# LIU-YUXI/SA-GNN

Measured on AMD Instinct MI355X. Metric: spmm_edges_per_sec, higher is better.
Workload: dtype f32

## Files before the change

sa-gnn_amd/csrc/attn_split.hip:

```cpp
#include "common.h"
#include "f16_split.h"

namespace {

typedef float f32x4 __attribute__((ext_vector_type(4)));
typedef int i32x4 __attribute__((ext_vector_type(4)));
typedef int i32x2 __attribute__((ext_vector_type(2)));

constexpr int kRows = 64;
constexpr int kBT = 4;
constexpr int kRec = 48;

template <int D>
__device__ __forceinline__ int swz(int row) {
  if (D == 128) return row & 15;
  if (D == 64) return (row >> 1) & 7;
  const int g = (row >> 2) & 3;
  return (0x78 >> (2 * g)) & 3;
}
__device__ __forceinline__ void lds_barrier() { asm volatile("s_waitcnt lgkmcnt(0)\n\ts_barrier" ::: "memory"); }

__host__ __device__ constexpr int pad_node(int t) { return t == 6 ? 16 : 0; }
__host__ __device__ constexpr int pad_group(int t) { return (t == 1 || t == 3 || t == 5) ? 64 : t == 6 ? 32 : 16; }
__host__ __device__ constexpr int lanes_per_pair(int t, int d) {
  if (d == 128) return (t % 4 == 0) ? 4 : (t % 2 == 0) ? 2 : 1;
  return t == 16 ? 4 : (t == 8 || t == 12) ? 2 : 1;
}

template <int DK>
struct HeadVec {
  typedef float type __attribute__((ext_vector_type(DK)));
  static __device__ __forceinline__ type load(const char* p, int gs) { return *reinterpret_cast<const type*>(p); }
  static __device__ __forceinline__ void store(char* p, int gs, type v) { *reinterpret_cast<type*>(p) = v; }
};
template <>
struct HeadVec<8> {
  typedef float type __attribute__((ext_vector_type(8)));
  typedef float f4 __attribute__((ext_vector_type(4)));
  static __device__ __forceinline__ type load(const char* p, int gs) {
    const f4 a = *reinterpret_cast<const f4*>(p), b = *reinterpret_cast<const f4*>(p + gs);
    return type{a[0], a[1], a[2], a[3], b[0], b[1], b[2], b[3]};
  }
  static __device__ __forceinline__ void store(char* p, int gs, type v) {
    *reinterpret_cast<f4*>(p) = f4{v[0], v[1], v[2], v[3]};
    *reinterpret_cast<f4*>(p + gs) = f4{v[4], v[5], v[6], v[7]};
  }
};

template <int CTRL>
__device__ __forceinline__ float dpp_add(float v) {
  return v + __builtin_bit_cast(float, __builtin_amdgcn_update_dpp(0, __builtin_bit_cast(int, v), CTRL, 0xf, 0xf, true));
}
template <int LPR>
__device__ __forceinline__ float row_sum(float v) {
  v = dpp_add<0xB1>(v);
  v = dpp_add<0x4E>(v);
  v = dpp_add<0x141>(v);
  if constexpr (LPR >= 16) v = dpp_add<0x140>(v);
  if constexpr (LPR == 32) v += __shfl_xor(v, 16);
  return v;
}

template <int D, int T, int LP, bool BWD>
__global__ __launch_bounds__(64 * (D >= 64 ? 4 : D / 16), (D == 128 || (BWD && T >= 8)) ? 1 : 2) void ln_mhsa_split_kernel(
    const float* __restrict__ x, int64_t ld_n, int64_t ld_t, int64_t n, const float* __restrict__ gamma,
    const float* __restrict__ beta, float eps, int apply_ln, const float* __restrict__ Wq,
    const float* __restrict__ bq, const float* __restrict__ Wk, const float* __restrict__ bk,
    const float* __restrict__ Wv, const float* __restrict__ bv, float* out, int64_t ld_out,
    int64_t n_tiles, float* __restrict__ dqkv_out, float* __restrict__ y_out, unsigned int* __restrict__ redo_ctr) {
  static_assert(!BWD || D <= 64 || LP == 1, "d = 128: the backward front keeps a pair in one lane");
  constexpr int NW = D >= 64 ? 4 : D / 16, NT = 64 * NW, KS = D / 32;
  constexpr int DK = D / 16;
  constexpr int HPW = 16 / DK;
  constexpr int NB = kRows / T;
  constexpr int ROWS = NB * T;
  constexpr int PLANE = kRows * D * 2;
  constexpr int LPR = D / 4, RPP = NT / LPR, NFILL = kRows / RPP;
  constexpr int PN = pad_node(T), PG = pad_group(T);
  constexpr int GS = kRows * kRec + NB * PN + PG;
  constexpr int QKVW = 4 * GS;
  typedef typename HeadVec<DK>::type vec;

  extern __shared__ __attribute__((aligned(16))) char lds[];
  char* const Yp = lds;
  char* const QKV = lds + 2 * PLANE;
  float2* const rstat = reinterpret_cast<float2*>(QKV + NW * QKVW);
  float2* const nstat = rstat + kRows;
  int* const flags = reinterpret_cast<int*>(nstat + NB);
  const int tid = threadIdx.x, lane = tid & 63;
  const int wave = __builtin_amdgcn_readfirstlane(tid >> 6);
  const int m = lane & 15, q = lane >> 4;
  const int cbase = 64 * (int)blockIdx.y + 16 * wave;
  const int col0 = cbase + 4 * q;
  const int fr = tid / LPR, fc4 = (tid % LPR) * 4;
  char* const tab = QKV + wave * QKVW;
  constexpr bool WL = D == 64 && (T & (T - 1)) == 0;
  constexpr int PP = T >= 4 ? T / 4 : 1;
  constexpr int GP = T >= 4 ? 4 : T;
  auto fill_row = [&](int p, int fr_now) { return WL ? 16 * wave + 4 * p + (lane >> 4) : p * RPP + fr_now; };

  float k4096 = 4096.f;
  asm volatile("" : "+v"(k4096));
  if (tid < 3) flags[tid] = 0;
  __syncthreads();
  const float qscale = 1.44269504088896340736f * (DK == 4 ? 0.5f : DK == 2 ? 0.70710678118654752440f : 0.35355339059327376220f);

  i32x4 wf[3][KS][2];
  {
    const float* const Ws[3] = {Wq, Wk, Wv};
    RangeTrack wr = range_init();
#pragma unroll
    for (int mat = 0; mat < 3; ++mat)
#pragma unroll
      for (int ks = 0; ks < KS; ++ks) {
        float wv[8];
#pragma unroll
        for (int j = 0; j < 8; ++j) wv[j] = Ws[mat][(size_t)(32 * ks + 8 * q + j) * D + cbase + m] * (mat == 0 ? qscale : 1.f);
        range_seg4(wr, wv[0], wv[1], wv[2], wv[3]);
        range_seg4(wr, wv[4], wv[5], wv[6], wv[7]);
#pragma unroll
        for (int e = 0; e < 4; ++e) {
          const int hd = head2(wv[2 * e], wv[2 * e + 1]);
          wf[mat][ks][0][e] = hd;
          wf[mat][ks][1][e] = tail2(hd, wv[2 * e], wv[2 * e + 1], k4096);
        }
      }
    if (range_bad(wr)) flags[2] = 1;
  }
  f32x4 bias3[3];
#pragma unroll
  for (int r = 0; r < 4; ++r) {
    bias3[0][r] = bq[col0 + r] * qscale;
    bias3[1][r] = bk[col0 + r];
    bias3[2][r] = bv[col0 + r];
  }
  float4 g4 = make_float4(1.f, 1.f, 1.f, 1.f), b4 = make_float4(0.f, 0.f, 0.f, 0.f);
  if (apply_ln) {
    g4 = *reinterpret_cast<const float4*>(gamma + fc4);
    b4 = *reinterpret_cast<const float4*>(beta + fc4);
  }
  const float inv_t = 1.f / (float)T;

  float4 xr[NFILL];
  auto fetch_tile = [&](int64_t tile) {
    const int64_t node0 = tile * NB;
#pragma unroll
    for (int p = 0; p < NFILL; ++p) {
      const int r = fill_row(p, fr);
      const int nb = r / T, ts = r - nb * T;
      xr[p] = make_float4(0.f, 0.f, 0.f, 0.f);
      if (tile < n_tiles && r < ROWS && node0 + nb < n)
        xr[p] = *reinterpret_cast<const float4*>(x + (node0 + nb) * ld_n + (int64_t)ts * ld_t + fc4);
    }
  };
  fetch_tile(blockIdx.x);

  int par = 0;
  for (int64_t tile = blockIdx.x; tile < n_tiles; tile += gridDim.x, par ^= 1) {
    const int64_t node0 = tile * NB;
    if (tid == 0) flags[par] = 0;
    int fr_ = fr, fc4_ = fc4, m_ = m, q_ = q;
    asm volatile("" : "+v"(fr_), "+v"(fc4_), "+v"(m_), "+v"(q_));

    float2 wst[NFILL];
    if constexpr (WL) {
      if (apply_ln) {
        float mr[NFILL], m2[NFILL];
#pragma unroll
        for (int p = 0; p < NFILL; ++p) {
          mr[p] = row_sum<LPR>((xr[p].x + xr[p].y) + (xr[p].z + xr[p].w)) * (1.f / (float)D);
          const float dx = xr[p].x - mr[p], dy = xr[p].y - mr[p], dz = xr[p].z - mr[p], dw = xr[p].w - mr[p];
          m2[p] = row_sum<LPR>((dx * dx + dy * dy) + (dz * dz + dw * dw));
        }
#pragma unroll
        for (int j = 0; j < NFILL / PP; ++j) {
          float sm = 0.f;
#pragma unroll
          for (int i = 0; i < PP; ++i) sm += mr[j * PP + i];
          if constexpr (GP >= 2) sm += __shfl_xor(sm, 16);
          if constexpr (GP == 4) sm += __shfl_xor(sm, 32);
          const float mean = sm * inv_t;
          float q2 = 0.f;
#pragma unroll
          for (int i = 0; i < PP; ++i) {
            const float dm = mr[j * PP + i] - mean;
            q2 += m2[j * PP + i] + (float)D * dm * dm;
          }
          if constexpr (GP >= 2) q2 += __shfl_xor(q2, 16);
          if constexpr (GP == 4) q2 += __shfl_xor(q2, 32);
          const float2 st = make_float2(mean, rsqrtf(q2 * (1.f / (float)(T * D)) + eps));
#pragma unroll
          for (int i = 0; i < PP; ++i) wst[j * PP + i] = st;
          const int r0 = fill_row(j * PP, fr_);
          if (fc4_ == 0 && r0 % T == 0) nstat[r0 / T] = st;
        }
      }
    } else if (apply_ln) {
#pragma unroll
      for (int p = 0; p < NFILL; ++p) {
        const float mr = row_sum<LPR>((xr[p].x + xr[p].y) + (xr[p].z + xr[p].w)) * (1.f / (float)D);
        const float dx = xr[p].x - mr, dy = xr[p].y - mr, dz = xr[p].z - mr, dw = xr[p].w - mr;
        const float m2 = row_sum<LPR>((dx * dx + dy * dy) + (dz * dz + dw * dw));
        if (fc4_ == 0) rstat[p * RPP + fr_] = make_float2(mr, m2);
      }
      lds_barrier();
      if (tid < NB) {
        float ms = 0.f;
#pragma unroll
        for (int ts = 0; ts < T; ++ts) ms += rstat[tid * T + ts].x;
        const float mean = ms * inv_t;
        float m2 = 0.f;
#pragma unroll
        for (int ts = 0; ts < T; ++ts) {
          const float2 st = rstat[tid * T + ts];
          const float dm = st.x - mean;
          m2 += st.y + (float)D * dm * dm;
        }
        nstat[tid] = make_float2(mean, rsqrtf(m2 * (1.f / (float)(T * D)) + eps));
      }
      lds_barrier();
    }
    RangeTrack yr = range_init();
#pragma unroll
    for (int p = 0; p < NFILL; ++p) {
      const int r = fill_row(p, fr_);
      float4 y = xr[p];
      if (apply_ln) {
        const float2 st = WL ? wst[p] : nstat[r < ROWS ? r / T : 0];
        const float ix = st.y * g4.x, iy = st.y * g4.y, iz = st.y * g4.z, iw = st.y * g4.w;
        y.x = xr[p].x * ix + (b4.x - st.x * ix);
        y.y = xr[p].y * iy + (b4.y - st.x * iy);
        y.z = xr[p].z * iz + (b4.z - st.x * iz);
        y.w = xr[p].w * iw + (b4.w - st.x * iw);
      }
      range_seg4(yr, y.x, y.y, y.z, y.w);
      if constexpr (BWD) {
        if (y_out && blockIdx.y == 0 && r < ROWS && node0 + r / T < n)
          *reinterpret_cast<float4*>(y_out + (node0 * T + r) * D + fc4_) = y;
      }
      const int p0 = head2(y.x, y.y), p1 = head2(y.z, y.w);
      const int off = r * (D * 2) + (((fc4_ >> 3) ^ swz<D>(r)) << 4) + ((fc4_ >> 2) & 1) * 8;
      *reinterpret_cast<i32x2*>(Yp + off) = i32x2{p0, p1};
      *reinterpret_cast<i32x2*>(Yp + PLANE + off) = i32x2{tail2(p0, y.x, y.y, k4096), tail2(p1, y.z, y.w, k4096)};
    }
    fetch_tile(tile + gridDim.x);
    lds_barrier();
    if (range_bad(yr)) flags[par] = 1;

#pragma unroll
    for (int bt = 0; bt < kBT; ++bt) {
      const int row = bt * 16 + m_;
      const int sw = swz<D>(row);
      f32x4 hi[3] = {bias3[0], bias3[1], bias3[2]};
      f32x4 lo[3];
#pragma unroll
      for (int ks = 0; ks < KS; ++ks) {
        const int off = row * (D * 2) + (((ks * 4 + q_) ^ sw) << 4);
        const f16x8 b1 = __builtin_bit_cast(f16x8, *reinterpret_cast<const i32x4*>(Yp + off));
        const f16x8 b2 = __builtin_bit_cast(f16x8, *reinterpret_cast<const i32x4*>(Yp + PLANE + off));
#pragma unroll
        for (int mat = 0; mat < 3; ++mat) {
          const f16x8 a1 = __builtin_bit_cast(f16x8, wf[mat][ks][0]);
          const f16x8 a2 = __builtin_bit_cast(f16x8, wf[mat][ks][1]);
          lo[mat] = __builtin_amdgcn_mfma_f32_16x16x32_f16(a2, b1, ks == 0 ? f32x4{0.f, 0.f, 0.f, 0.f} : lo[mat], 0, 0, 0);
          lo[mat] = __builtin_amdgcn_mfma_f32_16x16x32_f16(a1, b2, lo[mat], 0, 0, 0);
          hi[mat] = __builtin_amdgcn_mfma_f32_16x16x32_f16(a1, b1, hi[mat], 0, 0, 0);
        }
      }
      f32x4 acc[3];
#pragma unroll
      for (int mat = 0; mat < 3; ++mat)
#pragma unroll
        for (int r = 0; r < 4; ++r) acc[mat][r] = fmaf(lo[mat][r], kLoInv, hi[mat][r]);
      char* rec = tab + q_ * GS + row * kRec + (row / T) * PN;
      *reinterpret_cast<f32x4*>(rec) = acc[0];
      *reinterpret_cast<f32x4*>(rec + 16) = acc[1];
      *reinterpret_cast<f32x4*>(rec + 32) = acc[2];
    }
    lds_barrier();
    if (flags[par] | flags[2]) {
      if (tid == 0 && redo_ctr) atomicAdd(redo_ctr, 1u);
      constexpr int NCOL = 16 * NW;
      const float* const Ws[3] = {Wq, Wk, Wv};
      const float* const bs[3] = {bq, bk, bv};
      for (int idx = tid; idx < ROWS * 3 * NCOL; idx += NT) {
        const int r = idx / (3 * NCOL), rem = idx - r * (3 * NCOL), mat = rem / NCOL, cl = rem - mat * NCOL;
        const int nb = r / T, ts = r - nb * T;
        if (node0 + nb >= n) continue;
        const int col = 64 * (int)blockIdx.y + cl;
        const float sc = mat == 0 ? qscale : 1.f;
        const float2 st = apply_ln ? nstat[nb] : make_float2(0.f, 1.f);
        const float* const xrow = x + (node0 + nb) * ld_n + (int64_t)ts * ld_t;
        float acc = bs[mat][col] * sc;
        for (int k = 0; k < D; ++k) {
          float yv = xrow[k];
          if (apply_ln) {
            const float ik = st.y * gamma[k];
            yv = yv * ik + (beta[k] - st.x * ik);
          }
          acc = fmaf(yv, Ws[mat][(size_t)k * D + col] * sc, acc);
        }
        *reinterpret_cast<float*>(QKV + (cl >> 4) * QKVW + ((cl >> 2) & 3) * GS + r * kRec + nb * PN + mat * 16 + (cl & 3) * 4) = acc;
      }
      __syncthreads();
    }

    constexpr int PAIRS = NB * HPW;
    constexpr int LSTEP = 64 / LP;
    constexpr int TQ = T / LP;
    constexpr int KC = T <= 8 ? T : T / 2;
    static_assert(T % LP == 0 && T % KC == 0 && LP <= T, "query / key split");
    const int part = lane % LP;
    if constexpr (BWD) {
      const float scale = qscale * 0.69314718055994530942f;
      auto quad_sum = [&](float v) {
        if constexpr (LP > 1) v += __builtin_bit_cast(float, __builtin_amdgcn_update_dpp(0, __builtin_bit_cast(int, v), 0xB1, 0xf, 0xf, true));
        if constexpr (LP > 2) v += __builtin_bit_cast(float, __builtin_amdgcn_update_dpp(0, __builtin_bit_cast(int, v), 0x4E, 0xf, 0xf, true));
        return v;
      };
#pragma unroll 1
      for (int p = lane / LP; p < PAIRS; p += LSTEP) {
        const int hl = p % HPW, nb = p / HPW;
        const char* base = tab + ((hl * DK) >> 2) * GS + nb * (T * kRec + PN) + ((hl * DK) & 3) * 4;
        const int64_t node = node0 + nb;
        vec g = (vec)(0.f);
        if (node < n) g = *reinterpret_cast<const vec*>(out + node * ld_out + cbase + hl * DK);
        g *= inv_t;
        vec kv[T], vv[T], dk[T];
        float ps[T], asum[T];
#pragma unroll
        for (int ts = 0; ts < T; ++ts) {
          kv[ts] = HeadVec<DK>::load(base + ts * kRec + 16, GS);
          vv[ts] = HeadVec<DK>::load(base + ts * kRec + 32, GS);
          dk[ts] = (vec)(0.f);
          asum[ts] = 0.f;
          float pd = g[0] * vv[ts][0];
#pragma unroll
          for (int c = 1; c < DK; ++c) pd = fmaf(g[c], vv[ts][c], pd);
          ps[ts] = pd;
        }
        float* const drow = dqkv_out + (node * T) * (3 * D) + cbase + hl * DK;
#pragma unroll
        for (int i = 0; i < TQ; ++i) {
          const int tq = part * TQ + i;
          const vec qv = HeadVec<DK>::load(base + tq * kRec, GS);
          float a[T];
          float rs = 0.f;
#pragma unroll
          for (int s_ = 0; s_ < T; ++s_) {
            float z = qv[0] * kv[s_][0];
#pragma unroll
            for (int c = 1; c < DK; ++c) z = fmaf(qv[c], kv[s_][c], z);
            a[s_] = __builtin_amdgcn_exp2f(z);
            rs += a[s_];
          }
          const float inv = __builtin_amdgcn_rcpf(rs + 1e-8f);
          float dot = 0.f;
#pragma unroll
          for (int s_ = 0; s_ < T; ++s_) {
            a[s_] *= inv;
            dot = fmaf(a[s_], ps[s_], dot);
          }
          vec dq = (vec)(0.f);
#pragma unroll
          for (int s_ = 0; s_ < T; ++s_) {
            const float dz = a[s_] * (ps[s_] - dot);
            dq += dz * kv[s_];
            dk[s_] += dz * qv;
            asum[s_] += a[s_];
          }
          if (node < n) *reinterpret_cast<vec*>(drow + tq * (3 * D)) = dq * scale;
        }
        if constexpr (LP > 1) {
#pragma unroll
          for (int ts = 0; ts < T; ++ts) {
#pragma unroll
            for (int c = 0; c < DK; ++c) {
              float v = dk[ts][c];
              v = quad_sum(v);
              dk[ts][c] = v;
            }
            asum[ts] = quad_sum(asum[ts]);
          }
        }
        if (node < n) {
#pragma unroll
          for (int ts = 0; ts < T; ++ts) {
            if (LP > 1 && ts / TQ != part) continue;
            *reinterpret_cast<vec*>(drow + ts * (3 * D) + D) = dk[ts] * 0.69314718055994530942f;
            *reinterpret_cast<vec*>(drow + ts * (3 * D) + 2 * D) = g * asum[ts];
          }
        }
      }
      continue;
    }
#pragma unroll 1
    for (int p = lane / LP; p < PAIRS; p += LSTEP) {
      const int hl = p % HPW, nb = p / HPW;
      char* base = tab + ((hl * DK) >> 2) * GS + nb * (T * kRec + PN) + ((hl * DK) & 3) * 4;
      vec qv[TQ];
      float e[TQ][T], rs[TQ];
#pragma unroll
      for (int i = 0; i < TQ; ++i) qv[i] = HeadVec<DK>::load(base + (part * TQ + i) * kRec, GS);
#pragma unroll
      for (int ch = 0; ch < T / KC; ++ch) {
        vec k[KC];
#pragma unroll
        for (int s = 0; s < KC; ++s) k[s] = HeadVec<DK>::load(base + (ch * KC + s) * kRec + 16, GS);
#pragma unroll
        for (int i = 0; i < TQ; ++i)
#pragma unroll
          for (int s = 0; s < KC; ++s) {
            float pd = qv[i][0] * k[s][0];
#pragma unroll
            for (int c = 1; c < DK; ++c) pd = fmaf(qv[i][c], k[s][c], pd);
            const float ev = __builtin_amdgcn_exp2f(pd);
            e[i][ch * KC + s] = ev;
            rs[i] = (ch == 0 && s == 0) ? ev : rs[i] + ev;
          }
      }
      float w[T];
#pragma unroll
      for (int i = 0; i < TQ; ++i) {
        const float inv = __builtin_amdgcn_rcpf(rs[i] + 1e-8f);
#pragma unroll
        for (int s = 0; s < T; ++s) w[s] = i == 0 ? e[0][s] * inv : fmaf(e[i][s], inv, w[s]);
      }
      vec o = (vec)(0.f);
#pragma unroll
      for (int ch = 0; ch < T / KC; ++ch) {
        vec v[KC];
#pragma unroll
        for (int s = 0; s < KC; ++s) v[s] = HeadVec<DK>::load(base + (ch * KC + s) * kRec + 32, GS);
#pragma unroll
        for (int s = 0; s < KC; ++s) o += w[ch * KC + s] * v[s];
      }
      if (LP > 1) {
#pragma unroll
        for (int c = 0; c < DK; ++c) {
          float oc = o[c];
          oc += __builtin_bit_cast(float, __builtin_amdgcn_update_dpp(0, __builtin_bit_cast(int, oc), 0xB1, 0xf, 0xf, true));
          if (LP > 2) oc += __builtin_bit_cast(float, __builtin_amdgcn_update_dpp(0, __builtin_bit_cast(int, oc), 0x4E, 0xf, 0xf, true));
          o[c] = oc;
        }
      }
      const int64_t node = node0 + nb;
      if (part == 0 && node < n) {
        const vec ov = o * inv_t;
        float* dst = out + node * ld_out + cbase + hl * DK;
        if constexpr (DK == 8) {
          *reinterpret_cast<float4*>(dst) = make_float4(ov[0], ov[1], ov[2], ov[3]);
          *reinterpret_cast<float4*>(dst + 4) = make_float4(ov[4], ov[5], ov[6], ov[7]);
        } else {
          *reinterpret_cast<vec*>(dst) = ov;
        }
      }
    }
  }
}

}

namespace sagnn {

template <int D, int T, bool BWD>
static int launch_split(const SeqView& v, const AttnParams& a, float* out, int64_t ld_out, const AttnBwdOut& b, hipStream_t s) {
  constexpr int NW = D >= 64 ? 4 : D / 16, NB = kRows / T;
  constexpr int LP = (BWD && D == 128) ? 1 : lanes_per_pair(T, D);
  constexpr int GS = kRows * kRec + NB * pad_node(T) + pad_group(T);
  const size_t lds = (size_t)2 * kRows * D * 2 + (size_t)NW * 4 * GS + (size_t)(kRows + NB) * sizeof(float2) + 16;
  if (int rc = ensure_dynamic_lds(reinterpret_cast<const void*>(&ln_mhsa_split_kernel<D, T, LP, BWD>), lds)) return rc;
  const int per_cu = (D == 128 || (BWD && T >= 8)) ? 1 : D == 64 ? 2 : 4;
  constexpr int CB = D == 128 ? 2 : 1;
  const int64_t n_tiles = (v.n + NB - 1) / NB;
  const int64_t want = (int64_t)cu_count_current() * per_cu / CB;
  const int64_t blocks = n_tiles < want ? n_tiles : (want > 0 ? want : 1);
  ProfileScope prof(kProfMhsa, s, v.n, T);
  hipLaunchKernelGGL((ln_mhsa_split_kernel<D, T, LP, BWD>), dim3((unsigned)blocks, CB), dim3(64 * NW), lds, s, v.x, v.ld_n, v.ld_t,
                     v.n, a.gamma, a.beta, a.eps, a.apply_ln, a.Wq, a.bq, a.Wk, a.bk, a.Wv, a.bv,
                     BWD ? const_cast<float*>(b.g_out) : out, BWD ? b.ld_g : ld_out, n_tiles, b.dqkv, b.y, redo_counter());
  SAGNN_HIP_TRY(hipGetLastError());
  return SAGNN_OK;
}

template <int D>
static int ln_mhsa_mean_split_d(const SeqView& v, const AttnParams& a, float* out, int64_t ld_out, hipStream_t s) {
  int rc;
  const auto launch = [&](auto T) { return launch_split<D, decltype(T)::value, false>(v, a, out, ld_out, AttnBwdOut{}, s); };
  if (dispatch_t(v.t, SpecialisedT{}, launch, rc)) return rc;
  return fail(SAGNN_ERR_DIM, "split attention: t = %d has no specialised kernel", v.t);
}

int ln_mhsa_mean_split(const SeqView& v, const AttnParams& a, float* out, int64_t ld_out, hipStream_t s) {
  if (!mhsa_split_supported(v.d, v.t, a.heads)) return fail(SAGNN_ERR_DIM, "split attention: unsupported d/t/heads");
  if (v.d == 128) return ln_mhsa_mean_split_d<128>(v, a, out, ld_out, s);
  if (v.d == 64) return ln_mhsa_mean_split_d<64>(v, a, out, ld_out, s);
  return ln_mhsa_mean_split_d<32>(v, a, out, ld_out, s);
}

template <int D>
static int attn_bwd_front_split_d(const SeqView& v, const AttnParams& a, const AttnBwdOut& b, hipStream_t s) {
  using Ts = std::conditional_t<D == 128, SplitBwdFrontT128, SpecialisedT>;
  int rc;
  const auto launch = [&](auto T) { return launch_split<D, decltype(T)::value, true>(v, a, nullptr, 0, b, s); };
  if (dispatch_t(v.t, Ts{}, launch, rc)) return rc;
  return fail(SAGNN_ERR_DIM, "split attention backward front: t = %d has no specialised kernel", v.t);
}

int attn_bwd_front_split(const SeqView& v, const AttnParams& a, const AttnBwdOut& b, hipStream_t s) {
  if (!attn_bwd_front_split_supported(v.d, v.t, a.heads))
    return fail(SAGNN_ERR_DIM, "split attention backward front: unsupported d/t/heads");
  if (v.d == 128) return attn_bwd_front_split_d<128>(v, a, b, s);
  if (v.d == 64) return attn_bwd_front_split_d<64>(v, a, b, s);
  return attn_bwd_front_split_d<32>(v, a, b, s);
}

}
```

sa-gnn_amd/csrc/common.h:

```cpp
#pragma once
#include <hip/hip_runtime.h>
#include <stdint.h>
#include <stdio.h>
#include <string>

#include "engine.h"
#include "sagnn.h"

namespace sagnn {

std::string& last_error_slot();
int fail(int code, const char* fmt, ...) __attribute__((format(printf, 2, 3)));
int hip_fail(hipError_t e, const char* what);

inline bool aligned16(const void* p) { return (reinterpret_cast<uintptr_t>(p) & 15u) == 0; }

#define SAGNN_HIP_TRY(expr)                                   \
  do {                                                        \
    hipError_t _e = (expr);                                   \
    if (_e != hipSuccess) return ::sagnn::hip_fail(_e, #expr); \
  } while (0)

inline int lanes_per_row(int d) {
  int need = (d + 3) / 4;
  int lpr = 8;
  while (lpr < need) lpr <<= 1;
  return lpr;
}

int ensure_dynamic_lds(const void* kernel, size_t bytes);
int cu_count_current();
unsigned int* redo_counter();

struct SeqView {
  const float* x;
  int64_t ld_n, ld_t, n;
  int t, d;
  bool vec() const { return aligned16(x) && (ld_n & 3) == 0 && (ld_t & 3) == 0; }
};
struct AttnParams {
  int heads;
  const float *gamma, *beta;
  float eps;
  int apply_ln;
  const float *Wq, *bq, *Wk, *bk, *Wv, *bv;
};
struct AttnBwdOut {
  const float* g_out;
  int64_t ld_g;
  float *dqkv, *y;
};
struct LstmArgs {
  SeqView x;
  const float *W, *b;
  float forget_bias;
  const float* drop;
  float* h;
  int64_t ld_h;
  float *gates, *cell;
  const float* h_init;
  int64_t ld_hi;
  const float* c_init;
  float* c_final;
};

int lstm_fwd_mfma(const LstmArgs& a, hipStream_t s);
int ln_mhsa_mean_mfma(const SeqView& v, const AttnParams& a, float* out, int64_t ld_out, hipStream_t s);
int attn_bwd_front_mfma(const SeqView& v, const AttnParams& a, const AttnBwdOut& b, hipStream_t s);
int lstm_fwd_f16(const LstmArgs& a, hipStream_t s);
int ln_mhsa_mean_split(const SeqView& v, const AttnParams& a, float* out, int64_t ld_out, hipStream_t s);
int attn_bwd_front_split(const SeqView& v, const AttnParams& a, const AttnBwdOut& b, hipStream_t s);
int lstm_fwd_split128(const LstmArgs& a, hipStream_t s);
int attn_bwd_tail_f16(float* y, const float* dqkv, int64_t rows, int d, const float* Wqkv, float* dWqkv, float* dbqkv,
                      hipStream_t s);
int lstm_dw_f16(const float* x, int64_t ld_n, int64_t ld_t, const float* h, const float* dg, int64_t n, int t, int d, float* dW,
                hipStream_t s);
int dense_nn_any(const float* X, int64_t ldx, int64_t n, int din, int dout, const float* W, int64_t ldw,
                 const float* bias, float* Y, int64_t ldy, int accumulate, hipStream_t s);
int dense_tn_any(const float* X, int64_t ldx, const float* G, int64_t ldg, int64_t n, int din, int dout, float* dW,
                 int64_t lddw, float* db, hipStream_t s);
int gemm_nn(const float* X, int64_t ldx, int64_t n, int din, int dout, const float* W, int64_t ldw, const float* bias, float* Y,
            int64_t ldy, int accumulate, hipStream_t s);
int gemm_tn(const float* X, int64_t ldx, int64_t xseg, const float* G, int64_t ldg, int64_t gseg, int64_t seg_rows, int64_t n_seg,
            int din, int dout, float* dW, int64_t lddw, float* db, hipStream_t s);

enum ProfileKind { kProfSpmmRows = 0, kProfSpmmFixup = 1, kProfLstm = 2, kProfLayerNorm = 3, kProfMhsa = 4 };

class ProfileScope {
 public:
  ProfileScope(int kind, hipStream_t stream, int64_t units_a, int64_t units_b);
  ~ProfileScope();
  ProfileScope(const ProfileScope&) = delete;
  ProfileScope& operator=(const ProfileScope&) = delete;

 private:
  int slot_;
  hipStream_t stream_;
};

}
```

Measured before the change: 18.18 billion.

## Add specialised rows16 attention kernel for d=64, t=16 forward path

Adds a dedicated LayerNorm+MHSA mean kernel for d=64, t=16, 16 heads. Each wave holds one node's 16 timesteps and computes QKV with f16-split MFMA. Scores are formed with DPP row rotations in inline asm instead of going through LDS, and the kernel double-buffers tiles to run three workgroups per CU. Shared helpers move into a common header, and the split dispatcher routes this shape to the new kernel. This is aimed at the attention stage, which may not be what the spmm metric measures, and it adds hand-written asm with a fallback that recomputes when values fall out of range.

```diff
diff --git a/sa-gnn_amd/csrc/attn_rows16.hip b/sa-gnn_amd/csrc/attn_rows16.hip
--- /dev/null
+++ b/sa-gnn_amd/csrc/attn_rows16.hip
@@ -0,0 +1,276 @@
+#include "attn_split_common.h"
+
+#ifndef SAGNN_ROWS16_PER_CU
+#define SAGNN_ROWS16_PER_CU 3
+#endif
+
+namespace {
+
+constexpr int kD = 64, kT = 16;
+constexpr int kPlane = kRows * kD * 2;
+constexpr int kScratch = 3 * kT * kD * 4;
+constexpr int kLds = 4 * kPlane + kScratch + kBT * (int)sizeof(float2) + 16;
+constexpr int kLdsAsk = SAGNN_ROWS16_PER_CU >= 3 ? kLds : 160 * 1024 / (SAGNN_ROWS16_PER_CU + 1) + 1024;
+static_assert(kLdsAsk >= kLds && 3 * kLds <= 160 * 1024, "three workgroups per CU");
+
+template <int R>
+__device__ __forceinline__ float row_ror(float v) {
+  return __builtin_bit_cast(float, __builtin_amdgcn_update_dpp(0, __builtin_bit_cast(int, v), 0x120 + R, 0xf, 0xf, true));
+}
+
+#define SAGNN_DPP_ROW "row_mask:0xf bank_mask:0xf bound_ctrl:1\n\t"
+#define SAGNN_ROT_DOT(o, r)                                                  \
+  "v_mul_f32_dpp %" #o ", %15, %19 row_ror:" #r " " SAGNN_DPP_ROW            \
+  "v_fmac_f32_dpp %" #o ", %16, %20 row_ror:" #r " " SAGNN_DPP_ROW           \
+  "v_fmac_f32_dpp %" #o ", %17, %21 row_ror:" #r " " SAGNN_DPP_ROW           \
+  "v_fmac_f32_dpp %" #o ", %18, %22 row_ror:" #r " " SAGNN_DPP_ROW
+__device__ __forceinline__ void rotated_scores(const float (&q)[4], const float (&k)[4], float (&z)[kT]) {
+  z[0] = fmaf(k[3], q[3], fmaf(k[2], q[2], fmaf(k[1], q[1], k[0] * q[0])));
+  asm("s_nop 1\n\t"
+      SAGNN_ROT_DOT(0, 1) SAGNN_ROT_DOT(1, 2) SAGNN_ROT_DOT(2, 3) SAGNN_ROT_DOT(3, 4) SAGNN_ROT_DOT(4, 5)
+      SAGNN_ROT_DOT(5, 6) SAGNN_ROT_DOT(6, 7) SAGNN_ROT_DOT(7, 8) SAGNN_ROT_DOT(8, 9) SAGNN_ROT_DOT(9, 10)
+      SAGNN_ROT_DOT(10, 11) SAGNN_ROT_DOT(11, 12) SAGNN_ROT_DOT(12, 13) SAGNN_ROT_DOT(13, 14) SAGNN_ROT_DOT(14, 15)
+      : "=&v"(z[1]), "=&v"(z[2]), "=&v"(z[3]), "=&v"(z[4]), "=&v"(z[5]), "=&v"(z[6]), "=&v"(z[7]), "=&v"(z[8]), "=&v"(z[9]),
+        "=&v"(z[10]), "=&v"(z[11]), "=&v"(z[12]), "=&v"(z[13]), "=&v"(z[14]), "=&v"(z[15])
+      : "v"(k[0]), "v"(k[1]), "v"(k[2]), "v"(k[3]), "v"(q[0]), "v"(q[1]), "v"(q[2]), "v"(q[3]));
+}
+#undef SAGNN_ROT_DOT
+#undef SAGNN_DPP_ROW
+
+template <int... R>
+__device__ __forceinline__ float gather_weights(const float (&p)[kT], std::integer_sequence<int, R...>) {
+  float w = p[0];
+  ((w = row_ror<kT - 1 - R>(p[1 + R]) + w), ...);
+  return w;
+}
+__device__ __forceinline__ float key_weights(const float (&q)[4], const float (&k)[4]) {
+  float e[kT];
+  rotated_scores(q, k, e);
+  float rs = 0.f;
+#pragma unroll
+  for (int r = 0; r < kT; ++r) {
+    e[r] = __builtin_amdgcn_exp2f(e[r]);
+    rs = r == 0 ? e[0] : rs + e[r];
+  }
+  const float inv = __builtin_amdgcn_rcpf(rs + 1e-8f);
+#pragma unroll
+  for (int r = 0; r < kT; ++r) e[r] *= inv;
+  return gather_weights(e, std::make_integer_sequence<int, kT - 1>{});
+}
+
+__global__ __launch_bounds__(256, SAGNN_ROWS16_PER_CU) void ln_mhsa_rows16_kernel(
+    const float* __restrict__ x, int64_t ld_n, int64_t ld_t, int64_t n, const float* __restrict__ gamma,
+    const float* __restrict__ beta, float eps, int apply_ln, const float* __restrict__ Wq,
+    const float* __restrict__ bq, const float* __restrict__ Wk, const float* __restrict__ bk,
+    const float* __restrict__ Wv, const float* __restrict__ bv, float* out, int64_t ld_out,
+    int64_t n_tiles, unsigned int* __restrict__ redo_ctr) {
+  constexpr int D = kD, T = kT, KS = D / 32, NFILL = 4;
+
+  extern __shared__ __attribute__((aligned(16))) char lds[];
+  char* const Yp = lds;
+  float* const scratch = reinterpret_cast<float*>(lds + 4 * kPlane);
+  float2* const nstat = reinterpret_cast<float2*>(lds + 4 * kPlane + kScratch);
+  int* const flags = reinterpret_cast<int*>(nstat + kBT);
+  const int tid = threadIdx.x, lane = tid & 63;
+  const int wave = __builtin_amdgcn_readfirstlane(tid >> 6);
+  const int m = lane & 15, q = lane >> 4;
+  const int cbase = 16 * wave;
+  const int col0 = cbase + 4 * q;
+  const int fc4 = m * 4;
+
+  float k4096 = 4096.f;
+  asm volatile("" : "+v"(k4096));
+  if (tid < 4) flags[tid] = 0;
+  __syncthreads();
+  const float qscale = 1.44269504088896340736f * 0.5f;
+
+  i32x4 wf[3][KS][2];
+  {
+    const float* const Ws[3] = {Wq, Wk, Wv};
+    RangeTrack wr = range_init();
+#pragma unroll
+    for (int mat = 0; mat < 3; ++mat)
+#pragma unroll
+      for (int ks = 0; ks < KS; ++ks) {
+        float wv[8];
+#pragma unroll
+        for (int j = 0; j < 8; ++j) wv[j] = Ws[mat][(size_t)(32 * ks + 8 * q + j) * D + cbase + m] * (mat == 0 ? qscale : 1.f);
+        range_seg4(wr, wv[0], wv[1], wv[2], wv[3]);
+        range_seg4(wr, wv[4], wv[5], wv[6], wv[7]);
+#pragma unroll
+        for (int e = 0; e < 4; ++e) {
+          const int hd = head2(wv[2 * e], wv[2 * e + 1]);
+          wf[mat][ks][0][e] = hd;
+          wf[mat][ks][1][e] = tail2(hd, wv[2 * e], wv[2 * e + 1], k4096);
+        }
+      }
+    if (range_bad(wr)) flags[3] = 1;
+  }
+  f32x4 bias3[3];
+#pragma unroll
+  for (int r = 0; r < 4; ++r) {
+    bias3[0][r] = bq[col0 + r] * qscale;
+    bias3[1][r] = bk[col0 + r];
+    bias3[2][r] = bv[col0 + r];
+  }
+  float4 g4 = make_float4(1.f, 1.f, 1.f, 1.f), b4 = make_float4(0.f, 0.f, 0.f, 0.f);
+  if (apply_ln) {
+    g4 = *reinterpret_cast<const float4*>(gamma + fc4);
+    b4 = *reinterpret_cast<const float4*>(beta + fc4);
+  }
+  const float inv_t = 1.f / (float)T;
+
+  float4 xr[NFILL];
+  auto fetch_tile = [&](int64_t tile) {
+    const int64_t node = tile * kBT + wave;
+#pragma unroll
+    for (int p = 0; p < NFILL; ++p) {
+      xr[p] = make_float4(0.f, 0.f, 0.f, 0.f);
+      if (tile < n_tiles && node < n)
+        xr[p] = *reinterpret_cast<const float4*>(x + node * ld_n + (int64_t)(4 * p + q) * ld_t + fc4);
+    }
+  };
+  fetch_tile(blockIdx.x);
+
+  int par = 0, slot = 0;
+  for (int64_t tile = blockIdx.x; tile < n_tiles; tile += gridDim.x, par ^= 1, slot = slot == 2 ? 0 : slot + 1) {
+    const int64_t node0 = tile * kBT;
+    char* const Yt = Yp + par * (2 * kPlane);
+    int fc4_ = fc4, m_ = m, q_ = q;
+    asm volatile("" : "+v"(fc4_), "+v"(m_), "+v"(q_));
+
+    float2 st = make_float2(0.f, 1.f);
+    if (apply_ln) {
+      float mr[NFILL], m2[NFILL];
+#pragma unroll
+      for (int p = 0; p < NFILL; ++p) {
+        mr[p] = row_sum<16>((xr[p].x + xr[p].y) + (xr[p].z + xr[p].w)) * (1.f / (float)D);
+        const float dx = xr[p].x - mr[p], dy = xr[p].y - mr[p], dz = xr[p].z - mr[p], dw = xr[p].w - mr[p];
+        m2[p] = row_sum<16>((dx * dx + dy * dy) + (dz * dz + dw * dw));
+      }
+      float sm = 0.f;
+#pragma unroll
+      for (int i = 0; i < NFILL; ++i) sm += mr[i];
+      sm += __shfl_xor(sm, 16);
+      sm += __shfl_xor(sm, 32);
+      const float mean = sm * inv_t;
+      float q2 = 0.f;
+#pragma unroll
+      for (int i = 0; i < NFILL; ++i) {
+        const float dm = mr[i] - mean;
+        q2 += m2[i] + (float)D * dm * dm;
+      }
+      q2 += __shfl_xor(q2, 16);
+      q2 += __shfl_xor(q2, 32);
+      st = make_float2(mean, rsqrtf(q2 * (1.f / (float)(T * D)) + eps));
+      if (lane == 0) nstat[wave] = st;
+    }
+    RangeTrack yr = range_init();
+#pragma unroll
+    for (int p = 0; p < NFILL; ++p) {
+      const int r = 16 * wave + 4 * p + q_;
+      float4 y = xr[p];
+      if (apply_ln) {
+        const float ix = st.y * g4.x, iy = st.y * g4.y, iz = st.y * g4.z, iw = st.y * g4.w;
+        y.x = xr[p].x * ix + (b4.x - st.x * ix);
+        y.y = xr[p].y * iy + (b4.y - st.x * iy);
+        y.z = xr[p].z * iz + (b4.z - st.x * iz);
+        y.w = xr[p].w * iw + (b4.w - st.x * iw);
+      }
+      range_seg4(yr, y.x, y.y, y.z, y.w);
+      const int p0 = head2(y.x, y.y), p1 = head2(y.z, y.w);
+      const int off = r * (D * 2) + (((fc4_ >> 3) ^ swz<D>(r)) << 4) + ((fc4_ >> 2) & 1) * 8;
+      *reinterpret_cast<i32x2*>(Yt + off) = i32x2{p0, p1};
+      *reinterpret_cast<i32x2*>(Yt + kPlane + off) = i32x2{tail2(p0, y.x, y.y, k4096), tail2(p1, y.z, y.w, k4096)};
+    }
+    fetch_tile(tile + gridDim.x);
+    if (range_bad(yr)) flags[slot] = 1;
+    lds_barrier();
+    if (tid == 0) flags[slot == 0 ? 2 : slot - 1] = 0;
+    const bool redo = (flags[slot] | flags[3]) != 0;
+    if (redo && tid == 0 && redo_ctr) atomicAdd(redo_ctr, 1u);
+
+#pragma unroll 1
+    for (int bt = 0; bt < kBT; ++bt) {
+      const int64_t node = node0 + bt;
+      if (node >= n) break;
+      f32x4 acc[3];
+      if (!redo) {
+        const int row = bt * 16 + m_;
+        const int sw = swz<D>(row);
+        f32x4 hi[3] = {bias3[0], bias3[1], bias3[2]};
+        f32x4 lo[3];
+#pragma unroll
+        for (int ks = 0; ks < KS; ++ks) {
+          const int off = row * (D * 2) + (((ks * 4 + q_) ^ sw) << 4);
+          const f16x8 b1 = __builtin_bit_cast(f16x8, *reinterpret_cast<const i32x4*>(Yt + off));
+          const f16x8 b2 = __builtin_bit_cast(f16x8, *reinterpret_cast<const i32x4*>(Yt + kPlane + off));
+#pragma unroll
+          for (int mat = 0; mat < 3; ++mat) {
+            const f16x8 a1 = __builtin_bit_cast(f16x8, wf[mat][ks][0]);
+            const f16x8 a2 = __builtin_bit_cast(f16x8, wf[mat][ks][1]);
+            lo[mat] = __builtin_amdgcn_mfma_f32_16x16x32_f16(a2, b1, ks == 0 ? f32x4{0.f, 0.f, 0.f, 0.f} : lo[mat], 0, 0, 0);
+            lo[mat] = __builtin_amdgcn_mfma_f32_16x16x32_f16(a1, b2, lo[mat], 0, 0, 0);
+            hi[mat] = __builtin_amdgcn_mfma_f32_16x16x32_f16(a1, b1, hi[mat], 0, 0, 0);
+          }
+        }
+#pragma unroll
+        for (int mat = 0; mat < 3; ++mat)
+#pragma unroll
+          for (int r = 0; r < 4; ++r) acc[mat][r] = fmaf(lo[mat][r], kLoInv, hi[mat][r]);
+      } else {
+        const float* const Ws[3] = {Wq, Wk, Wv};
+        const float* const bs[3] = {bq, bk, bv};
+        const float2 ns = apply_ln ? nstat[bt] : make_float2(0.f, 1.f);
+        __syncthreads();
+        for (int idx = tid; idx < T * 3 * D; idx += 256) {
+          const int ts = idx / (3 * D), rem = idx - ts * (3 * D), mat = rem / D, col = rem - mat * D;
+          const float sc = mat == 0 ? qscale : 1.f;
+          const float* const xrow = x + node * ld_n + (int64_t)ts * ld_t;
+          float a = bs[mat][col] * sc;
+          for (int k = 0; k < D; ++k) {
+            float yv = xrow[k];
+            if (apply_ln) {
+              const float ik = ns.y * gamma[k];
+              yv = yv * ik + (beta[k] - ns.x * ik);
+            }
+            a = fmaf(yv, Ws[mat][(size_t)k * D + col] * sc, a);
+          }
+          scratch[(mat * T + ts) * D + col] = a;
+        }
+        __syncthreads();
+#pragma unroll
+        for (int mat = 0; mat < 3; ++mat) acc[mat] = *reinterpret_cast<const f32x4*>(scratch + (mat * T + m_) * D + col0);
+      }
+
+      const float qv[4] = {acc[0][0], acc[0][1], acc[0][2], acc[0][3]};
+      const float kv[4] = {acc[1][0], acc[1][1], acc[1][2], acc[1][3]};
+      const float w = key_weights(qv, kv) * inv_t;
+      float4 o;
+      o.x = row_sum<16>(w * acc[2][0]);
+      o.y = row_sum<16>(w * acc[2][1]);
+      o.z = row_sum<16>(w * acc[2][2]);
+      o.w = row_sum<16>(w * acc[2][3]);
+      if (m_ == 0) *reinterpret_cast<float4*>(out + node * ld_out + col0) = o;
+    }
+  }
+}
+
+}
+
+namespace sagnn {
+
+int ln_mhsa_mean_rows16(const SeqView& v, const AttnParams& a, float* out, int64_t ld_out, hipStream_t s) {
+  if (v.d != kD || v.t != kT || a.heads != 16) return fail(SAGNN_ERR_DIM, "rows16 attention: d = 64, t = 16, 16 heads only");
+  if (int rc = ensure_dynamic_lds(reinterpret_cast<const void*>(&ln_mhsa_rows16_kernel), kLdsAsk)) return rc;
+  const int64_t n_tiles = (v.n + kBT - 1) / kBT;
+  const int64_t want = (int64_t)cu_count_current() * SAGNN_ROWS16_PER_CU;
+  const int64_t blocks = n_tiles < want ? n_tiles : (want > 0 ? want : 1);
+  ProfileScope prof(kProfMhsa, s, v.n, kT);
+  hipLaunchKernelGGL(ln_mhsa_rows16_kernel, dim3((unsigned)blocks), dim3(256), kLdsAsk, s, v.x, v.ld_n, v.ld_t, v.n, a.gamma, a.beta,
+                     a.eps, a.apply_ln, a.Wq, a.bq, a.Wk, a.bk, a.Wv, a.bv, out, ld_out, n_tiles, redo_counter());
+  SAGNN_HIP_TRY(hipGetLastError());
+  return SAGNN_OK;
+}
+
+}
diff --git a/sa-gnn_amd/csrc/attn_split.hip b/sa-gnn_amd/csrc/attn_split.hip
--- a/sa-gnn_amd/csrc/attn_split.hip
+++ b/sa-gnn_amd/csrc/attn_split.hip
@@ -1,24 +1,8 @@
-#include "common.h"
-#include "f16_split.h"
+#include "attn_split_common.h"
 
 namespace {
 
-typedef float f32x4 __attribute__((ext_vector_type(4)));
-typedef int i32x4 __attribute__((ext_vector_type(4)));
-typedef int i32x2 __attribute__((ext_vector_type(2)));
-
-constexpr int kRows = 64;
-constexpr int kBT = 4;
 constexpr int kRec = 48;
-
-template <int D>
-__device__ __forceinline__ int swz(int row) {
-  if (D == 128) return row & 15;
-  if (D == 64) return (row >> 1) & 7;
-  const int g = (row >> 2) & 3;
-  return (0x78 >> (2 * g)) & 3;
-}
-__device__ __forceinline__ void lds_barrier() { asm volatile("s_waitcnt lgkmcnt(0)\n\ts_barrier" ::: "memory"); }
 
 __host__ __device__ constexpr int pad_node(int t) { return t == 6 ? 16 : 0; }
 __host__ __device__ constexpr int pad_group(int t) { return (t == 1 || t == 3 || t == 5) ? 64 : t == 6 ? 32 : 16; }
@@ -46,20 +30,6 @@
     *reinterpret_cast<f4*>(p + gs) = f4{v[4], v[5], v[6], v[7]};
   }
 };
-
-template <int CTRL>
-__device__ __forceinline__ float dpp_add(float v) {
-  return v + __builtin_bit_cast(float, __builtin_amdgcn_update_dpp(0, __builtin_bit_cast(int, v), CTRL, 0xf, 0xf, true));
-}
-template <int LPR>
-__device__ __forceinline__ float row_sum(float v) {
-  v = dpp_add<0xB1>(v);
-  v = dpp_add<0x4E>(v);
-  v = dpp_add<0x141>(v);
-  if constexpr (LPR >= 16) v = dpp_add<0x140>(v);
-  if constexpr (LPR == 32) v += __shfl_xor(v, 16);
-  return v;
-}
 
 template <int D, int T, int LP, bool BWD>
 __global__ __launch_bounds__(64 * (D >= 64 ? 4 : D / 16), (D == 128 || (BWD && T >= 8)) ? 1 : 2) void ln_mhsa_split_kernel(
@@ -486,6 +456,7 @@
 template <int D>
 static int ln_mhsa_mean_split_d(const SeqView& v, const AttnParams& a, float* out, int64_t ld_out, hipStream_t s) {
   int rc;
+  if (D == 64 && v.t == 16) return ln_mhsa_mean_rows16(v, a, out, ld_out, s);
   const auto launch = [&](auto T) { return launch_split<D, decltype(T)::value, false>(v, a, out, ld_out, AttnBwdOut{}, s); };
   if (dispatch_t(v.t, SpecialisedT{}, launch, rc)) return rc;
   return fail(SAGNN_ERR_DIM, "split attention: t = %d has no specialised kernel", v.t);
diff --git a/sa-gnn_amd/csrc/attn_split_common.h b/sa-gnn_amd/csrc/attn_split_common.h
--- /dev/null
+++ b/sa-gnn_amd/csrc/attn_split_common.h
@@ -0,0 +1,37 @@
+#pragma once
+#include "common.h"
+#include "f16_split.h"
+
+namespace {
+
+typedef float f32x4 __attribute__((ext_vector_type(4)));
+typedef int i32x4 __attribute__((ext_vector_type(4)));
+typedef int i32x2 __attribute__((ext_vector_type(2)));
+
+constexpr int kRows = 64;
+constexpr int kBT = 4;
+
+template <int D>
+__device__ __forceinline__ int swz(int row) {
+  if (D == 128) return row & 15;
+  if (D == 64) return (row >> 1) & 7;
+  const int g = (row >> 2) & 3;
+  return (0x78 >> (2 * g)) & 3;
+}
+__device__ __forceinline__ void lds_barrier() { asm volatile("s_waitcnt lgkmcnt(0)\n\ts_barrier" ::: "memory"); }
+
+template <int CTRL>
+__device__ __forceinline__ float dpp_add(float v) {
+  return v + __builtin_bit_cast(float, __builtin_amdgcn_update_dpp(0, __builtin_bit_cast(int, v), CTRL, 0xf, 0xf, true));
+}
+template <int LPR>
+__device__ __forceinline__ float row_sum(float v) {
+  v = dpp_add<0xB1>(v);
+  v = dpp_add<0x4E>(v);
+  v = dpp_add<0x141>(v);
+  if constexpr (LPR >= 16) v = dpp_add<0x140>(v);
+  if constexpr (LPR == 32) v += __shfl_xor(v, 16);
+  return v;
+}
+
+}
diff --git a/sa-gnn_amd/csrc/common.h b/sa-gnn_amd/csrc/common.h
--- a/sa-gnn_amd/csrc/common.h
+++ b/sa-gnn_amd/csrc/common.h
@@ -70,6 +70,7 @@
 int lstm_fwd_f16(const LstmArgs& a, hipStream_t s);
 int ln_mhsa_mean_split(const SeqView& v, const AttnParams& a, float* out, int64_t ld_out, hipStream_t s);
 int attn_bwd_front_split(const SeqView& v, const AttnParams& a, const AttnBwdOut& b, hipStream_t s);
+int ln_mhsa_mean_rows16(const SeqView& v, const AttnParams& a, float* out, int64_t ld_out, hipStream_t s);
 int lstm_fwd_split128(const LstmArgs& a, hipStream_t s);
 int attn_bwd_tail_f16(float* y, const float* dqkv, int64_t rows, int d, const float* Wqkv, float* dWqkv, float* dbqkv,
                       hipStream_t s);
```

Result: slower. 17.99 billion (-1.1%).
